# angelini/raft-simulation

Hardware: AMD Instinct MI355X
Metric: simulated node-ticks/sec (5-node Raft) (higher is better)
Workload: dtype u32; 1 GPU; C2: 65,536 5-node clusters/GPU, 10k ticks/step, no faults, no client (steady window); clusters=65536, clusters_per_gpu=65536, nodes=5, parallelism=cluster-sharded x1

## Files before the change

### raft-simulation_amd/csrc/steady_kernel.hip

```cpp
#include <hip/hip_ext.h>

#include "fixed_point_affine.hpp"
#include "tick_wave.hpp"

namespace rs {

constexpr int LANE_WG = 256;

__device__ __forceinline__ uint32_t msel(bool a, uint32_t x, uint32_t y) {
  const uint32_t m = 0u - (uint32_t)a;
  return (x & m) | (y & ~m);
}

constexpr int IMG_SLOTS = 32;
constexpr uint32_t IMG_LINE = 64 * 8 * 16;
constexpr uint32_t IMG_HALF = 2 * IMG_LINE;
constexpr uint32_t IMG_WAVE = 2 * IMG_HALF;
__device__ __forceinline__ uint32_t img_sw(uint32_t l) { return (l ^ (l >> 3)) & 7u; }
__device__ __forceinline__ uint32_t img_off(uint32_t l, uint32_t i) {
  return i < 16 ? (i >> 3) * IMG_LINE + l * 128u + 16u * ((i & 7u) ^ img_sw(l))
                : IMG_HALF + l * 256u + 16u * ((i & 15u) ^ (l & 15u));
}
template <typename T>
__device__ __forceinline__ T* lds_at(char* img, uint32_t off) {
// ... 49 lines not shown
  return SetWords{vreg(c.lead.a), vreg(c.lead.x), vreg(c.lead.y), vreg(c.lead.z),
                  vreg(c.fol.a),  vreg(c.fol.x),  vreg(c.fol.y),  vreg(c.fol.z),
                  vreg(c.lead.s), vreg(c.fol.s),  vreg(c.K),      vreg(K1)};
}
template <int I>
__device__ __forceinline__ void park_lane(uint32_t& park, uint32_t v) {
  asm volatile("v_writelane_b32 %0, %1, %2"
               : "+v"(park)
               : "s"(__builtin_amdgcn_readfirstlane(v)), "n"(I));
}
template <int F>
__device__ __forceinline__ fpa::Band band_sets(uint32_t nt, uint32_t d, uint32_t hb, BandSets* out) {
  const fpa::Band b = fpa::band(F, d, hb, nt);
  const uint32_t K1 = b.K1;
  const fpa::Set lo = fpa::build<F>(d, hb, K1 ? K1 - 1 : 0), hi = fpa::step<F>(lo, d, hb);
  out->k[0] = vreg(lo, K1);
  out->k[1] = vreg(hi, K1);
  return b;
}

template <int N>
struct FixedPoint {
  static constexpr int F = N - 1;
  static constexpr bool IN_BAND = false;
  uint32_t L, Lid, Lterm, Lcommit;
  uint64_t Ltr, ftr[F];
  uint32_t Ldl, fdl[F], fpend;
  uint32_t qmask, qA[F], qT[F], qa[F], qb[F];
  uint32_t rmask, resA, rT[F], rA[F], rB[F], rH[F];
  uint32_t nhb, nae, nar;

  __device__ __forceinline__ uint32_t fk(int j) const { return (uint32_t)j + ((uint32_t)j >= L ? 1u : 0u); }

  __device__ __forceinline__ void append_entries(uint32_t ta, uint32_t d, uint32_t el_base) {
#pragma unroll
    for (int j = 0; j < F; ++j) {
      ftr[j] = trace_event(ftr[j], ta, RAFT_MSG_APPEND_ENTRIES, Lid, Lterm, RAFT_FOLLWER, Lterm, 0);
      fdl[j] = ta + el_base;
      rT[j] = Lterm; rA[j] = Lcommit; rB[j] = 0; rH[j] = 1;
      qA[j] = INF;
    }
    fpend = (1u << F) - 1;
    qmask = 0;
    rmask = (1u << F) - 1;
    resA = ta + d;
    nae += F;
  }
  __device__ __forceinline__ void responses(uint32_t th, uint32_t tend, uint32_t d, uint32_t hb) {
#pragma unroll
    for (int j = 0; j < F; ++j) {
      const uint32_t tau = th + 2 * d + j;
      if (((rmask >> j) & 1) && tau < tend) {
        Ltr = trace_event(Ltr, tau, RAFT_MSG_APPEND_RESPONSE, fk(j) + 1, Lterm, RAFT_LEADER,
                          Lterm, 0);
        rmask &= ~(1u << j);
        Ldl = tau + hb;
        ++nar;
      }
    }
    if (!rmask) resA = INF;
  }
  __device__ __forceinline__ uint32_t term() const { return Lterm; }
  __device__ __forceinline__ uint32_t sid(int j) const { return fk(j) + 1; }
  __device__ __forceinline__ void followers(uint64_t a, uint64_t add) {
#pragma unroll
    for (int j = 0; j < F; ++j) ftr[j] = ftr[j] * a + add;
  }
  __device__ __forceinline__ void rearmed(uint32_t v) {
#pragma unroll
    for (int j = 0; j < F; ++j) fdl[j] = v;
    fpend = (1u << F) - 1;
  }
  __device__ __forceinline__ void heartbeat(uint32_t ta) {
#pragma unroll
    for (int j = 0; j < F; ++j) {
      qA[j] = ta; qT[j] = Lterm; qa[j] = Lcommit; qb[j] = 0;
    }
    qmask = (1u << F) - 1;
  }
  __device__ __forceinline__ bool queued() const { return rmask != 0; }

  __device__ __forceinline__ int slot(int k) const {
    return (uint32_t)k > L ? (k > 0 ? k - 1 : 0) : (k < F ? k : F - 1);
  }
  __device__ __forceinline__ uint32_t at_node(const uint32_t (&x)[F], int k) const {
    return msel((uint32_t)k > L, x[k > 0 ? k - 1 : 0], x[k < F ? k : F - 1]);
  }
  template <int NV>
  __device__ __forceinline__ void node_words(int k, uint32_t (&v)[NV][N]) const {
    const bool isL = (uint32_t)k == L;
    const int jl = k > 0 ? k - 1 : 0, jh = k < F ? k : F - 1;
    const bool lo = (uint32_t)k > L;
    const uint32_t fq = (qmask >> slot(k)) & 1, fqa = at_node(qA, k);
    const uint64_t trf = (uint64_t)msel(lo, (uint32_t)(ftr[jl] >> 32), (uint32_t)(ftr[jh] >> 32)) << 32 |
                         msel(lo, (uint32_t)ftr[jl], (uint32_t)ftr[jh]);
    const uint64_t tr = isL ? Ltr : trf;
    v[HF_DEADLINE][k] = isL ? Ldl : at_node(fdl, k);
    v[HF_TRACE_LO][k] = (uint32_t)tr;
    v[HF_TRACE_HI][k] = (uint32_t)(tr >> 32);
    v[HF_QMETA][k] = isL ? pack_qmeta(0, 0, 0, __popc(rmask)) : pack_qmeta(0, fq, 0, 0);
    v[HF_REQ_ARR][k] = isL ? INF : (fq ? fqa : INF);
    v[HF_RES_ARR][k] = isL ? resA : INF;
    v[HF_REQ_TAIL][k] = isL ? 0u : (fq ? fqa : 0u);
    v[HF_RES_TAIL][k] = isL ? (rmask ? resA : 0u) : 0u;
  }
  __device__ __forceinline__ void to_rings(const DevSim& S, uint32_t c, bool on) const {
    if (!__builtin_amdgcn_ballot_w64(on && (qmask || rmask))) return;
#pragma unroll
    for (int j = 0; j < F; ++j) {
      if (on && ((qmask >> j) & 1)) {
        uint4* dp = reinterpret_cast<uint4*>(qslots(S, c * N + fk(j), 0));
        dp[0] = make_uint4(qA[j], RAFT_MSG_APPEND_ENTRIES | Lid << 3, qT[j], qa[j]);
        dp[1] = make_uint4(qb[j], 0, 0, 0);
      }
    }
    uint4* rp = reinterpret_cast<uint4*>(qslots(S, c * N + L, 1));
    uint32_t n = 0;
#pragma unroll
    for (int j = 0; j < F; ++j) {
      if (on && ((rmask >> j) & 1)) {
        uint4* dp = rp + 2 * n;
        dp[0] = make_uint4(resA, RAFT_MSG_APPEND_RESPONSE | sid(j) << 3 | rH[j] << 7, rT[j], rA[j]);
        dp[1] = make_uint4(rB[j], 0, 0, 0);
        ++n;
      }
    }
  }
};

template <int N>
struct NodeOrder {
  static constexpr int F = N - 1;
  static constexpr bool IN_BAND = true;
  uint32_t L, T;
  uint64_t tr[N], Ltr;
  uint32_t Ldl;
  bool qin, took;
  uint32_t qA, fdl;
  uint32_t rc, resA;
  uint32_t nhb, nae, nar;

  __device__ __forceinline__ uint32_t sid(int j) const {
    return (uint32_t)j + 1 + ((uint32_t)j >= L ? 1u : 0u);
  }
  __device__ __forceinline__ void followers(uint64_t a, uint64_t add) {
#pragma unroll
    for (int k = 0; k < N; ++k) tr[k] = tr[k] * a + add;
  }
  __device__ __forceinline__ void append_entries(uint32_t ta, uint32_t d, uint32_t el_base) {
    followers(TRACE_M2, trace_term(ta, RAFT_MSG_APPEND_ENTRIES, L + 1, T, RAFT_FOLLWER, T, 0));
    took = true;
    fdl = ta + el_base;
    qin = false;
    rc = F;
    resA = ta + d;
    nae += F;
  }
  __device__ __forceinline__ void responses(uint32_t th, uint32_t tend, uint32_t d, uint32_t hb) {
#pragma unroll
    for (int j = 0; j < F; ++j) {
      const uint32_t tau = th + 2 * d + j;
      if ((uint32_t)j + rc >= (uint32_t)F && tau < tend) {
        Ltr = trace_event(Ltr, tau, RAFT_MSG_APPEND_RESPONSE, sid(j), T, RAFT_LEADER, T, 0);
        --rc;
        Ldl = tau + hb;
        ++nar;
      }
    }
    if (!rc) resA = INF;
  }
  __device__ __forceinline__ uint32_t term() const { return T; }
  __device__ __forceinline__ void rearmed(uint32_t v) { took = true; fdl = v; }
  __device__ __forceinline__ void heartbeat(uint32_t ta) { qin = true; qA = ta; }
  __device__ __forceinline__ bool queued() const { return rc != 0; }
};

struct LaunchBand {
  uint32_t t0;
  fpa::Band b;
};
template <typename St>
__device__ __forceinline__ void rounds(St& s, uint32_t th, uint32_t tend, uint32_t d, uint32_t hb,
                                       uint32_t el_base, const BandSets& bs, const LaunchBand& lb) {
  constexpr int F = St::F;
  const uint32_t P = 2 * d + F - 1 + hb, last = 2 * d + F - 1, T = s.term();
  uint32_t K, tk;
  if constexpr (St::IN_BAND) {
    const uint32_t delta = th - lb.t0;
    K = fpa::band_rounds(lb.b, delta);
    tk = th + fpa::band_ticks(lb.b, P, delta);
    const SetWords sw = bs.k[(delta <= lb.b.rho) & (lb.b.K1 != 0)];
    const fpa::Half cl = sw.lead(), cf = sw.fol();
    s.Ltr = fpa::apply_leader<F>(cl, s.Ltr, th, T, s.L);
    s.followers(cf.a, fpa::follower_addend<F>(cf, th, T, s.L));
    if (K) {
      s.rearmed(tk - P + d + el_base);
      s.Ldl = tk;
      s.nhb += K;
      s.nae += F * K;
      s.nar += F * K;
    }
  } else {
    K = tend > th + last ? (tend - th - last - 1) / P + 1 : 0;
    tk = th + K * P;
  }
  if (!St::IN_BAND && K) {
    const uint32_t K1 = bs.k[0].K1;
    const bool top = K == K1;
    if (!__builtin_amdgcn_ballot_w64(!top && K + 1 != K1)) {
      const SetWords sw = bs.k[top];
      const fpa::Half cl = sw.lead(), cf = sw.fol();
      s.Ltr = fpa::apply_leader<F>(cl, s.Ltr, th, T, s.L);
      s.followers(cf.a, fpa::follower_addend<F>(cf, th, T, s.L));
    } else {
      uint64_t a = trace_term(th, 7, 0, 0, RAFT_LEADER, T, 0);
#pragma unroll
      for (int j = 0; j < F; ++j)
        a = a * TRACE_M2 + trace_term(th + 2 * d + j, RAFT_MSG_APPEND_RESPONSE, s.sid(j), T,
                                      RAFT_LEADER, T, 0);
      const uint64_t da = (uint64_t)P * (TRACE_M * trace_geo<F + 1>());
      const uint64_t df = (uint64_t)P * TRACE_M;
      uint64_t cf = trace_term(th + d, RAFT_MSG_APPEND_ENTRIES, s.L + 1, T, RAFT_FOLLWER, T, 0);
      for (uint32_t r = 0; r < K; ++r) {
        s.Ltr = s.Ltr * trace_pow<F + 1>() + a;
        a += da;
        s.followers(TRACE_M2, cf);
        cf += df;
      }
    }
    s.rearmed(tk - P + d + el_base);
    s.Ldl = tk;
    s.nhb += K;
    s.nae += F * K;
    s.nar += F * K;
  }
  if (tk < tend) {
    s.Ltr = trace_event(s.Ltr, tk, 7, 0, 0, RAFT_LEADER, T, 0);
    ++s.nhb;
    s.Ldl = tk + hb;
    s.heartbeat(tk + d);
    if (tk + d < tend) {
      s.append_entries(tk + d, d, el_base);
      s.responses(tk, tend, d, hb);
    }
  }
}

template <typename St>
__device__ __forceinline__ void run_launch(St& s, uint32_t mid, uint32_t th0, uint32_t tend,
                                           uint32_t d, uint32_t hb, uint32_t el_base, uint32_t P,
                                           const BandSets& bs, const LaunchBand& lb) {
  bool whole = true;
  if (mid == 1) {
    if (th0 + d < tend) s.append_entries(th0 + d, d, el_base);
    else whole = false;
  }
  if (mid && whole) {
    s.responses(th0, tend, d, hb);
    whole = !s.queued();
  }
  if (whole) rounds(s, mid ? th0 + P : th0, tend, d, hb, el_base, bs, lb);
}

struct Schedule {
  uint32_t mid, th0, nxt;
  bool on;
};
template <int F>
__device__ __forceinline__ Schedule schedule(uint32_t t0, uint32_t tend, uint32_t d, uint32_t hb,
                                             uint32_t P, uint32_t Ldl, bool req, uint32_t reqA,
                                             uint32_t nres, uint32_t resA) {
  Schedule s{0, Ldl, 0, true};
  if (req) {
    s.mid = 1;
    s.th0 = reqA - d;
    s.on = reqA >= t0 && reqA >= d && Ldl == s.th0 + hb;
  } else if (nres) {
    s.mid = 2;
    s.th0 = resA - 2 * d;
    const uint32_t j0 = (uint32_t)F - nres;
    const int64_t cut = (int64_t)t0 - ((int64_t)s.th0 + 2 * d);
    s.on = resA >= 2 * d && (int64_t)j0 == (cut < 0 ? 0 : cut > F ? (int64_t)F : cut) &&
           Ldl == (j0 ? s.th0 + 2 * d + j0 - 1 : s.th0) + hb;
  } else {
    s.on = Ldl >= t0;
  }
  s.nxt = min((s.mid == 2 ? s.th0 + P : s.th0) + d, tend);
  return s;
}


template <int N>
__global__ void __launch_bounds__(LANE_WG) steady_lane_kernel(DevSim S, uint32_t t0, uint32_t nt) {
  static_assert(N >= 2 && N <= 5, "follower masks and the response queue fit four followers");
  constexpr int F = N - 1;
  constexpr uint32_t HB = hot_block_words(N);
  constexpr int NWORDS = (int)(HOT_CW + hf_abase(N) * N);
  constexpr int NW4 = (NWORDS + 3) / 4;
  constexpr int IMGC = (int)(HB / 4) < IMG_SLOTS ? (int)(HB / 4) : IMG_SLOTS;
  static_assert(NW4 <= IMGC && IMGC % 8 == 0, "the image holds the words read, in whole lines");
  __shared__ uint32_t bl_c[LANE_WG], bl_t[LANE_WG];
  __shared__ BandSets bs_keep[LANE_WG / 64];
  extern __shared__ __attribute__((aligned(16))) uint32_t dsm[];
  const uint32_t lane = threadIdx.x & 63, wave = threadIdx.x >> 6;
  const uint32_t cbase = blockIdx.x * LANE_WG + wave * 64;
  const uint32_t c0 = cbase + lane < S.C ? cbase + lane : INF;
  const bool active = c0 != INF;
  const uint32_t c = active ? c0 : 0u;
  const uint32_t g = S.goff + c;
  char* const img = reinterpret_cast<char*>(dsm) + wave * IMG_WAVE;
  uint32_t* const blc = bl_c + wave * 64;
  uint32_t* const blt = bl_t + wave * 64;
  uint32_t nbw = 0;
  auto record_bail = [&](bool b, uint32_t tick) {
    const uint64_t m = __builtin_amdgcn_ballot_w64(b);
    if (b) {
      const uint32_t i = nbw + __builtin_amdgcn_mbcnt_hi((uint32_t)(m >> 32),
                                                         __builtin_amdgcn_mbcnt_lo((uint32_t)m, 0u));
      blc[i] = c;
      blt[i] = tick;
    }
    nbw += (uint32_t)__popcll(m);
  };
#ifdef RS_WAVELOG
  const uint64_t wl_start = wall_clock64();
  uint32_t wl_trips = 0, wl_first = 0, wl_ph[6] = {0, 0, 0, 0, 0, 0};
  uint64_t wl_loop = 0, wl_ts = 0;
#define RS_LPH(i)                                         \
  do {                                                    \
    const uint64_t now_ = __builtin_amdgcn_s_memtime();   \
    wl_ph[i] += (uint32_t)(now_ - wl_ts);                 \
    wl_ts = now_;                                         \
  } while (0)
#else
#define RS_LPH(i) do {} while (0)
#endif

  auto load_wait = [&]() {
    asm volatile("s_waitcnt vmcnt(0)" ::: "memory");
  };
  auto load_line = [&](int ln, bool wait) {
    const uint32_t p = lane & 7;
#pragma unroll
    for (int j = 0; j < 8; ++j) {
      const uint32_t cc = 8 * j + (lane >> 3);
      const uint32_t i = 8 * ln + (p ^ img_sw(cc));
      const uint32_t cg = min(cbase + cc, S.C - 1);
      __builtin_amdgcn_global_load_lds(
          (const __attribute__((address_space(1))) void*)(S.hot + (size_t)cg * HB + 4 * i),
          (__attribute__((address_space(3))) void*)(img + ln * IMG_LINE + j * 1024), 16, 0, 0);
    }
    if (wait) load_wait();
  };
  auto load_half1 = [&]() {
    const uint32_t p = lane & 15;
#pragma unroll
    for (int j = 0; j < 16; ++j) {
      const uint32_t cc = 4 * j + (lane >> 4);
      const uint32_t i = 16 + (p ^ (cc & 15u));
      const uint32_t cg = min(cbase + cc, S.C - 1);
      if (i < (uint32_t)IMGC)
        __builtin_amdgcn_global_load_lds(
            (const __attribute__((address_space(1))) void*)(S.hot + (size_t)cg * HB + 4 * i),
            (__attribute__((address_space(3))) void*)(img + IMG_HALF + j * 1024), 16, 0, 0);
    }
    asm volatile("s_waitcnt vmcnt(0)" ::: "memory");
  };
  static_assert(IMGC >= 16, "lines 0 and 1 are whole in every block");
  uint32_t w[NW4 * 4];
  auto read_chunks = [&](int lo, int hi) {
#pragma unroll
    for (int i = lo; i < hi; ++i) {
      const uint4 x = *lds_at<const uint4>(img, img_off(lane, i));
      w[4 * i] = x.x; w[4 * i + 1] = x.y; w[4 * i + 2] = x.z; w[4 * i + 3] = x.w;
    }
  };
  auto word = [&](int f, int k) { return w[HOT_CW + f * N + k]; };
  auto lword = [&](int f, uint32_t L) {
    uint32_t v = 0;
#pragma unroll
    for (int k = 0; k < N; ++k) v |= word(f, k) & (0u - (uint32_t)(L == (uint32_t)k));
    return v;
  };
  auto fword = [&](int f, int j, uint32_t L) {
    return msel((uint32_t)j >= L, word(f, j + 1), word(f, j));
  };
  static_assert(HF_RES_TAIL + 1 == HF_FLAGS && (HOT_CW + HF_FLAGS * N) % 4 == 0 && HOT_CW % 4 == 0,
                "the fields written: DEADLINE .. RES_TAIL, whole chunks");
  constexpr int CH_END = (int)(HOT_CW + HF_FLAGS * N) / 4;
  asm volatile("" ::"s"(nt), "s"(t0), "s"(S.dmin), "s"(S.hb), "s"(S.el_base));
  load_line(0, false);
  const bool reporter = blockIdx.x == 0 && threadIdx.x == 0;
  uint32_t prev_bails = 0;
  if (reporter) prev_bails = *S.nbail_zero;
  uint32_t nt_s = nt;
  asm volatile("" : "+s"(nt_s));
  const BandSets& bs = bs_keep[wave];
  uint32_t park = 0;
  {
    const fpa::Band b = band_sets<F>(nt_s, S.dmin, S.hb, &bs_keep[wave]);
    park_lane<0>(park, b.K1);
    park_lane<1>(park, b.rho);
    park_lane<2>(park, b.K1P);
  }
  load_wait();
  asm volatile("" : "+v"(park));
  auto parked_band = [&]() {
    return fpa::Band{(uint32_t)__builtin_amdgcn_readlane(park, 0),
                     (uint32_t)__builtin_amdgcn_readlane(park, 1),
                     (uint32_t)__builtin_amdgcn_readlane(park, 2)};
  };
  if (reporter && prev_bails) {
    if (S.bail_report) *S.bail_report = prev_bails;
    *S.nbail_zero = 0;
  }
  static_assert(NW4 >= 8, "line 0 is read whole");
  read_chunks(0, 8);
  const uint32_t tend = t0 + nt, d = S.dmin, hb = S.hb, el_base = S.el_base;
  const uint32_t P = 2 * d + F - 1 + hb, allF = (1u << F) - 1;
  uint32_t dl = 0, nhb = 0, nae = 0, nar = 0;
  bool el = false;
  uint32_t el_to = 0;
#ifdef RS_WAVELOG
  uint64_t wl_x1 = 0, wl_x2 = 0, wl_x3 = 0, wl_lend = 0;
  uint32_t wl_cut = 0;
  asm volatile("" ::"v"(w[CL_CERT]), "v"(w[HOT_CW]));
  wl_loop = wall_clock64();
#endif

  static_assert(HOT_CW + (HF_QMETA + 1) * N <= 32 && HF_DEADLINE < HF_QMETA &&
                    HF_TRACE_LO < HF_QMETA && HF_TRACE_HI < HF_QMETA && CL_CTERM < HOT_CW,
                "every word the line-0 path reads is in line 0; REQ_ARR, RES_ARR, the flags and "
                "the term are derived (device.hpp)");
  NodeOrder<N> no;
  uint32_t lmid = 0, lth0 = 0;
  const bool cfg_ok = el_base >= P && hb >= 2 * d + F && S.Q >= (uint32_t)F;
  bool strong = active & cfg_ok & ((w[CL_CERT] & 0xFFFF0000u) == CERT_STRONG) &
                ((w[CL_CERT] & 0xFFFFu) < (uint32_t)N);
  {
    const uint32_t L = w[CL_CERT] & 0xFFFFu;
    no.L = L; no.T = w[CL_CTERM];
    no.Ldl = lword(HF_DEADLINE, L);
    no.Ltr = (uint64_t)lword(HF_TRACE_HI, L) << 32 | lword(HF_TRACE_LO, L);
#pragma unroll
    for (int k = 0; k < N; ++k) no.tr[k] = (uint64_t)word(HF_TRACE_HI, k) << 32 | word(HF_TRACE_LO, k);
    no.took = false; no.fdl = 0;
    no.nhb = no.nae = no.nar = 0;
    const uint32_t Lqm = lword(HF_QMETA, L), rsc = qm_res_cnt(Lqm);
    const uint32_t qm0 = L ? word(HF_QMETA, 0) : word(HF_QMETA, 1);
    const bool need = qm0 != 0;
    const bool cutr = !need & (rsc != 0);
    const uint32_t one_req = pack_qmeta(0, 1, 0, 0), only_res = pack_qmeta(0, 0, 0, rsc);
    strong = strong & ((qm0 & ~one_req) == 0) & (Lqm == only_res) & (rsc <= (uint32_t)F) &
             !(need & (rsc != 0));
#pragma unroll
    for (int k = 0; k < N; ++k) strong = strong & ((L == (uint32_t)k) | (word(HF_QMETA, k) == qm0));
    const uint32_t j0 = (uint32_t)F - rsc;
    const uint32_t back = msel(need | cutr, hb + msel(cutr & (j0 != 0), 2 * d + j0 - 1, 0u), 0u);
    lmid = msel(need, 1u, msel(cutr, 2u, 0u));
    lth0 = no.Ldl - back;
    const uint32_t ta = lth0 + d, ra = lth0 + 2 * d;
    const int64_t cut = (int64_t)t0 - (int64_t)ra;
    const bool on_need = ta >= t0;
    const bool on_cut = (int64_t)j0 == (cut < 0 ? 0 : cut > F ? (int64_t)F : cut);
    const bool on_none = no.Ldl >= t0;
    strong = strong & (no.Ldl >= back) & (need ? on_need : cutr ? on_cut : on_none);
    no.qin = need;
    no.qA = msel(need, ta, 0u);
    no.rc = msel(cutr, rsc, 0u);
    no.resA = msel(cutr, ra, INF);
    const uint32_t nxt = min(msel(cutr, lth0 + P, lth0) + d, tend);
#pragma unroll
    for (int k = 0; k < N; ++k)
      strong = strong & ((L == (uint32_t)k) | (word(HF_DEADLINE, k) >= nxt));
    strong = strong & (msel(lmid != 0, lth0 + P, lth0) - t0 < P);
  }
  const bool line0_wave = !__builtin_amdgcn_ballot_w64(active && !strong);
  if (line0_wave) {
#ifdef RS_WAVELOG
    asm volatile("" ::"v"(no.Ltr), "v"(no.Ldl), "v"(no.tr[0]), "v"(lth0));
    wl_x1 = wl_x2 = wall_clock64();
#endif
    if (active) {
      const LaunchBand lb{t0, parked_band()};
      run_launch(no, lmid, lth0, tend, d, hb, el_base, P, bs, lb);
      nhb = no.nhb; nae = no.nae; nar = no.nar;
#ifdef RS_WAVELOG
      asm volatile("" ::"v"(no.Ltr), "v"(no.tr[0]), "v"(no.Ldl));
      wl_x3 = wall_clock64();
#endif
      const uint32_t fqm = pack_qmeta(0, no.qin ? 1u : 0u, 0, 0), Lqm = pack_qmeta(0, 0, 0, no.rc);
      const uint32_t fra = no.qin ? no.qA : INF, frt = no.qin ? no.qA : 0u;
      const uint32_t Lrt = no.rc ? no.resA : 0u;
      auto val = [&](int q) -> uint32_t {
        const int f = (q - (int)HOT_CW) / N, k = (q - (int)HOT_CW) % N;
        const bool isL = no.L == (uint32_t)k;
        switch (f) {
          case HF_DEADLINE: return isL ? no.Ldl : no.took ? no.fdl : w[q];
          case HF_TRACE_LO: return (uint32_t)(isL ? no.Ltr : no.tr[k]);
          case HF_TRACE_HI: return (uint32_t)((isL ? no.Ltr : no.tr[k]) >> 32);
          case HF_QMETA: return isL ? Lqm : fqm;
          case HF_REQ_ARR: return isL ? INF : fra;
          case HF_RES_ARR: return isL ? no.resA : INF;
          case HF_REQ_TAIL: return isL ? 0u : frt;
          default: return isL ? Lrt : 0u;
        }
      };
      auto chunk = [&](int i) {
        return make_uint4(val(4 * i), val(4 * i + 1), val(4 * i + 2), val(4 * i + 3));
      };
#pragma unroll
      for (int i = (int)HOT_CW / 4; i < (CH_END < 8 ? CH_END : 8); ++i)
        *lds_at<uint4>(img, img_off(lane, i)) = chunk(i);
      dl = (nhb | nae | nar) != 0;
      if (CH_END > 8 && (lmid || no.qin || no.rc)) {
        uint4* const bp = reinterpret_cast<uint4*>(S.hot + (size_t)c * HB);
#pragma unroll
        for (int i = 8; i < CH_END; ++i) bp[i] = chunk(i);
      }
    }
    if (__builtin_amdgcn_ballot_w64(active && (no.qin || no.rc))) {
      if (active && no.qin) {
#pragma unroll
        for (int k = 0; k < N; ++k) {
          if (no.L != (uint32_t)k) {
            uint4* dp = reinterpret_cast<uint4*>(qslots(S, c * N + k, 0));
            dp[0] = make_uint4(no.qA, RAFT_MSG_APPEND_ENTRIES | (no.L + 1) << 3, no.T, 0);
            dp[1] = make_uint4(0, 0, 0, 0);
          }
        }
      }
      uint4* rp = reinterpret_cast<uint4*>(qslots(S, c * N + no.L, 1));
      uint32_t n = 0;
#pragma unroll
      for (int j = 0; j < F; ++j) {
        if (active && (uint32_t)j + no.rc >= (uint32_t)F) {
          uint4* dp = rp + 2 * n;
          dp[0] = make_uint4(no.resA, RAFT_MSG_APPEND_RESPONSE | no.sid(j) << 3 | 1u << 7, no.T, 0);
          dp[1] = make_uint4(0, 0, 0, 0);
          ++n;
        }
      }
    }
#ifdef RS_WAVELOG
    wl_lend = wall_clock64();
    wl_cut = __builtin_amdgcn_ballot_w64(active && (lmid || no.qin || no.rc)) ? 1u : 0u;
#endif
  }

  uint32_t Lc = 0;
  bool cert = false, full = false;
  if (!line0_wave) {
    load_line(1, true);
#pragma unroll
    for (int i = 32; i < NW4 * 4; ++i) w[i] = 0;
    read_chunks(8, NW4 < 16 ? NW4 : 16);
    uint32_t nlc = 0;
#pragma unroll
    for (int k = 0; k < N; ++k) {
      const bool lead = fl_role(w[HOT_CW + HF_FLAGS * N + k]) == RAFT_LEADER;
      Lc = lead ? (uint32_t)k : Lc;
      nlc += lead;
    }
    static_assert(HOT_CW + (HF_FLAGS + 1) * N <= 64, "the flags are in the first two lines");
    cert = active && nlc == 1 &&
           (w[CL_CERT] == (CERT_MAGIC | Lc) || w[CL_CERT] == (CERT_STRONG | Lc));
    full = IMGC > 16 && __builtin_amdgcn_ballot_w64(active && !cert) != 0;
    if (full) {
      load_half1();
      read_chunks(16, NW4);
    }
  }
  const bool vouched = cert && !full;

  FixedPoint<N> fx;
  const LaunchBand no_band{t0, fpa::Band{0, 0, 0}};
  bool lean = false;
  if (!line0_wave) {
    lean = vouched && cfg_ok;
    const uint32_t L = Lc;
    fx.L = L; fx.Lid = L + 1; fx.Lterm = lword(HF_TERM, L); fx.Lcommit = 0;
    fx.Ldl = lword(HF_DEADLINE, L);
    fx.Ltr = (uint64_t)lword(HF_TRACE_HI, L) << 32 | lword(HF_TRACE_LO, L);
    fx.qmask = fx.rmask = 0; fx.resA = INF; fx.fpend = allF; fx.nhb = fx.nae = fx.nar = 0;
    const uint32_t Lqm = lword(HF_QMETA, L);
    const uint32_t rsc = qm_res_cnt(Lqm);
    uint32_t need = 0;
#pragma unroll
    for (int j = 0; j < F; ++j) {
      fx.fdl[j] = fword(HF_DEADLINE, j, L);
      fx.ftr[j] = (uint64_t)fword(HF_TRACE_HI, j, L) << 32 | fword(HF_TRACE_LO, j, L);
      const uint32_t qm = fword(HF_QMETA, j, L);
      lean = lean && (fword(HF_FLAGS, j, L) & FL_DRAW) && ((qm >> 4) & 31) <= 1 && !qm_res_cnt(qm);
      need |= (qm_req_cnt(qm) ? 1u : 0u) << j;
      fx.qA[j] = INF; fx.qT[j] = fx.qa[j] = fx.qb[j] = 0;
      fx.rT[j] = fx.rA[j] = fx.rB[j] = fx.rH[j] = 0;
    }
    lean = lean && !qm_req_cnt(Lqm) && rsc <= (uint32_t)F && !(need && rsc) &&
           (need == 0 || need == allF);
    const uint32_t ta = fword(HF_REQ_ARR, 0, L), ra = lword(HF_RES_ARR, L);
    const Schedule sc = schedule<F>(t0, tend, d, hb, P, fx.Ldl, need != 0, ta, rsc, ra);
    lean = lean && sc.on;
    lmid = sc.mid;
    lth0 = sc.th0;
    if (lmid == 1) {
#pragma unroll
      for (int j = 0; j < F; ++j) {
        lean = lean && fword(HF_REQ_ARR, j, L) == ta;
        fx.qA[j] = ta; fx.qT[j] = fx.Lterm;
      }
      fx.qmask = allF;
    } else if (lmid == 2) {
      fx.rmask = allF & ~((1u << ((uint32_t)F - rsc)) - 1);
      fx.resA = ra;
#pragma unroll
      for (int j = 0; j < F; ++j) {
        fx.rT[j] = fx.Lterm; fx.rH[j] = 1;
      }
    }
#pragma unroll
    for (int j = 0; j < F; ++j) lean = lean && fx.fdl[j] >= sc.nxt;
  }
  const bool lean_wave = !line0_wave && !__builtin_amdgcn_ballot_w64(active && !lean);
  bool wb = false;
  if (lean_wave) {
#ifdef RS_WAVELOG
    asm volatile("" ::"v"(fx.Ltr), "v"(fx.fdl[0]), "v"(fx.ftr[0]), "v"(lth0));
    wl_x1 = wl_x2 = wall_clock64();
#endif
    if (active) {
      run_launch(fx, lmid, lth0, tend, d, hb, el_base, P, bs, no_band);
      nhb = fx.nhb; nae = fx.nae; nar = fx.nar;
#ifdef RS_WAVELOG
      asm volatile("" ::"v"(fx.Ltr), "v"(fx.ftr[0]), "v"(fx.Ldl));
      wl_x3 = wall_clock64();
#endif
      uint32_t v[HF_FLAGS][N];
#pragma unroll
      for (int k = 0; k < N; ++k) fx.node_words(k, v);
      auto val = [&](int q) { return v[(q - HOT_CW) / N][(q - HOT_CW) % N]; };
      auto chunk = [&](int i) {
        return make_uint4(val(4 * i), val(4 * i + 1), val(4 * i + 2), val(4 * i + 3));
      };
#pragma unroll
      for (int i = (int)HOT_CW / 4; i < CH_END; ++i) {
        const int q = 4 * i;
        const uint4 x = chunk(i);
        *lds_at<uint4>(img, img_off(lane, i)) = x;
        dl |= (uint32_t)(x.x != w[q] || x.y != w[q + 1] || x.z != w[q + 2] || x.w != w[q + 3])
              << (i / 8);
      }
      const uint32_t cn = CERT_STRONG | fx.L;
      *lds_at<uint4>(img, img_off(lane, CL_CERT / 4)) =
          make_uint4(w[CL_CERT - 3], w[CL_CERT - 2], fx.Lterm, cn);
      static_assert(CL_CTERM == CL_CERT - 1 && CL_CERT % 4 == 3, "one chunk");
      dl |= (uint32_t)(cn != w[CL_CERT] || fx.Lterm != w[CL_CTERM]);
    }
    fx.to_rings(S, c, active);
#ifdef RS_WAVELOG
    wl_lend = wall_clock64();
#endif
  } else if (!line0_wave) {
#ifdef RS_WAVELOG
    wl_loop = wall_clock64();
#endif
    {
      auto ifield = [&](int f, int k) { return w[HOT_CW + f * N + k]; };
      bool pat = active && w[CL_HWM_IDX] == 0 && S.Q >= 2u * F && el_base >= P && hb >= 2 * d + F;
      const uint32_t T = ifield(HF_TERM, 0);
#pragma unroll
      for (int k = 0; k < N; ++k) {
        pat = pat && ifield(HF_FLAGS, k) == 0 && ifield(HF_MASKS, k) == 0 &&
              ifield(HF_TERM, k) == T && ifield(HF_COMMIT, k) == 0 && ifield(HF_LEN, k) == 0 &&
              ifield(HF_QMETA, k) == 0 && ifield(HF_REQ_ARR, k) == INF &&
              ifield(HF_RES_ARR, k) == INF;
#pragma unroll
        for (int p = 0; p < 2 * N; ++p) pat = pat && ifield(HF_NEXT + p, k) == 0;
      }
      pat = pat && T != INF;
      uint32_t cidx = 0, t1 = INF, ntie = 0, bidx = 0;
#pragma unroll
      for (int k = 0; k < N; ++k) {
        const uint32_t dk = ifield(HF_DEADLINE, k);
        cidx = dk < t1 ? (uint32_t)k : cidx;
        t1 = min(t1, dk);
      }
      bool single = true;
#pragma unroll
      for (int k = 0; k < N; ++k) {
        const uint32_t dk = ifield(HF_DEADLINE, k);
        ntie += dk == t1;
        bidx = dk == t1 && (uint32_t)k != cidx ? (uint32_t)k : bidx;
        single = single && ((uint32_t)k == cidx || (uint64_t)dk >= (uint64_t)t1 + d);
      }
      const bool tie = ntie == 2 && d == 1 && N >= 3;
      constexpr uint32_t iL = (N + 1) / 2 >= 2 ? (N + 1) / 2 - 2 : 0;
      const uint64_t tL = (uint64_t)t1 + 2 * d + iL;
      const uint64_t tau0 = max((uint64_t)t1 + 2 * d + F, tL + 2 * d);
      const uint64_t tlast = tau0 + F - 1;
      pat = pat && (single || tie) && t1 >= t0 && (tie || tlast < tend) &&
            (uint64_t)t1 + 4 * N + 8 < 0xFFFFFFFFull;
      if (__builtin_amdgcn_ballot_w64(pat)) {
        const uint32_t* lp = S.hot + (size_t)c * HB + HOT_CW + hf_led(N) * N;
        uint32_t led[N];
#pragma unroll
        for (int k = 0; k < N; ++k) led[k] = lp[k];
#pragma unroll
        for (int k = 0; k < N; ++k) pat = pat && ((uint32_t)k == cidx || led[k] != T + 1);
      }
      const uint32_t T1 = T + 1, cid = cidx + 1, peers = ((1u << (N + 1)) - 1) & ~1u & ~(1u << cid);
      if (pat && single) {
        el = true;
        el_to = 1;
        uint64_t hc = 0;
#pragma unroll
        for (int k = 0; k < N; ++k)
          if ((uint32_t)k == cidx)
            hc = (uint64_t)ifield(HF_TRACE_HI, k) << 32 | ifield(HF_TRACE_LO, k);
        hc = trace_event(hc, t1, 6, 0, 0, RAFT_CANDIDATE, T1, 0);
#pragma unroll
        for (int i = 0; i < F; ++i) {
          const uint32_t sid = (uint32_t)i + ((uint32_t)i >= cidx ? 2u : 1u);
          hc = trace_event(hc, t1 + 2 * d + i, RAFT_MSG_VOTE_RESPONSE, sid, T,
                           (uint32_t)i >= iL ? RAFT_LEADER : RAFT_CANDIDATE, T1, 0);
        }
#pragma unroll
        for (int j = 0; j < F; ++j) {
          const uint32_t sid = (uint32_t)j + ((uint32_t)j >= cidx ? 2u : 1u);
          hc = trace_event(hc, (uint32_t)tau0 + j, RAFT_MSG_APPEND_RESPONSE, sid, T, RAFT_LEADER,
                           T1, 0);
        }
#pragma unroll
        for (int k = 0; k < N; ++k) {
          const bool isc = (uint32_t)k == cidx;
          uint64_t h = (uint64_t)ifield(HF_TRACE_HI, k) << 32 | ifield(HF_TRACE_LO, k);
          h = trace_event(h, t1 + d, RAFT_MSG_REQUEST_VOTE, cid, T1, RAFT_FOLLOWER, T, 0);
          h = trace_event(h, (uint32_t)tL + d, RAFT_MSG_APPEND_ENTRIES, cid, T1, RAFT_FOLLWER, T1, 0);
          h = isc ? hc : h;
          w[HOT_CW + HF_FLAGS * N + k] = isc ? pack_flags(RAFT_LEADER, 0, cid, 0, 0, 1)
                                             : pack_flags(RAFT_FOLLWER, 0, cid, 0, 0, 0) | FL_DRAW;
          w[HOT_CW + HF_MASKS * N + k] = isc ? peers << 16 : 0u;
          w[HOT_CW + HF_TERM * N + k] = T1;
          w[HOT_CW + HF_DEADLINE * N + k] = isc ? (uint32_t)tlast + hb
                                                : (uint32_t)tL + d + el_base;
          w[HOT_CW + HF_REQ_TAIL * N + k] = 0;
          w[HOT_CW + HF_RES_TAIL * N + k] = 0;
          w[HOT_CW + HF_TRACE_LO * N + k] = (uint32_t)h;
          w[HOT_CW + HF_TRACE_HI * N + k] = (uint32_t)(h >> 32);
        }
        nae = F;
        nar = F;
      } else if (pat && tie) {
        const uint32_t a = cidx, b = bidx, B = b + 1;
        const uint32_t A = cid;
        constexpr uint32_t M = (N + 1) / 2;
        uint64_t ha = 0, hbb = 0;
#pragma unroll
        for (int k = 0; k < N; ++k) {
          const uint64_t h0 = (uint64_t)ifield(HF_TRACE_HI, k) << 32 | ifield(HF_TRACE_LO, k);
          if ((uint32_t)k == a) ha = h0;
          if ((uint32_t)k == b) hbb = h0;
        }
        ha = trace_event(ha, t1, 6, 0, 0, RAFT_CANDIDATE, T1, 0);
        ha = trace_event(ha, t1 + 1, RAFT_MSG_REQUEST_VOTE, B, T1, RAFT_CANDIDATE, T1, 0);
        uint32_t votes = 1, tLt = INF, role = RAFT_CANDIDATE;
#pragma unroll
        for (int k = 0; k < N; ++k) {
          if ((uint32_t)k == a) continue;
          const uint32_t i = (uint32_t)k - ((uint32_t)k > a ? 1u : 0u), tau = t1 + 2 + i;
          const bool grant = (uint32_t)k != b;
          if (grant && role == RAFT_CANDIDATE && ++votes >= M) {
            role = RAFT_LEADER;
            tLt = tau;
          }
          ha = trace_event(ha, tau, RAFT_MSG_VOTE_RESPONSE, (uint32_t)k + 1, grant ? T : T1, role,
                           T1, 0);
        }
        hbb = trace_event(hbb, t1, 6, 0, 0, RAFT_CANDIDATE, T1, 0);
        hbb = trace_event(hbb, t1 + 1, RAFT_MSG_REQUEST_VOTE, A, T1, RAFT_CANDIDATE, T1, 0);
        hbb = trace_event(hbb, t1 + 2, RAFT_MSG_VOTE_RESPONSE, A, T1, RAFT_CANDIDATE, T1, 0);
        uint32_t tb = t1 + 3, j = 0, tbae = INF, brole = RAFT_CANDIDATE, bdl = 0;
        bool bexact = false;
        for (int it = 0; it < N + 1; ++it) {
          const bool res = j < (uint32_t)N - 2, req = tbae == INF;
          if (!res && !req) break;
          if (!res && tb < tLt + 1) tb = tLt + 1;
          const bool rq = req && tb >= tLt + 1;
          bool take_req = rq;
          bexact = false;
          if (res && rq) {
            const uint4 ew = event_draw(g, B, tb, S);
            take_req = !(ew.x & 1);
            bexact = true;
            bdl = tb + el_base + __umulhi(ew.y, S.el_span);
          }
          if (take_req) {
            hbb = trace_event(hbb, tb, RAFT_MSG_APPEND_ENTRIES, A, T1, RAFT_FOLLWER, T1, 0);
            brole = RAFT_FOLLWER;
            tbae = tb;
          } else {
            uint32_t fid = 0, cnt = 0;
#pragma unroll
            for (int k = 0; k < N; ++k) {
              const bool other = (uint32_t)k != a && (uint32_t)k != b;
              fid = other && cnt == j ? (uint32_t)k + 1 : fid;
              cnt += other;
            }
            hbb = trace_event(hbb, tb, RAFT_MSG_VOTE_RESPONSE, fid, T, brole, T1, 0);
            ++j;
          }
          if (!bexact) bdl = tb + el_base;
          ++tb;
        }
        const uint32_t tbl = tb - 1;
        uint32_t ta = t1 + N + 1;
        const uint32_t fa = tLt + 2, ba = tbae + 1;
#pragma unroll
        for (int k = 0; k < N; ++k) {
          if ((uint32_t)k == a) continue;
          const bool isb = (uint32_t)k == b;
          if (isb && ba != fa) continue;
          ta = max(ta, fa);
          ha = trace_event(ha, ta, RAFT_MSG_APPEND_RESPONSE, (uint32_t)k + 1, isb ? T1 : T,
                           RAFT_LEADER, T1, 0);
          ++ta;
        }
        if (ba != fa) {
          ta = max(ta, ba);
          ha = trace_event(ha, ta, RAFT_MSG_APPEND_RESPONSE, B, T1, RAFT_LEADER, T1, 0);
          ++ta;
        }
        const uint32_t tal = ta - 1;
        if (tbae != INF && tLt != INF && max(tal, tbl) < tend) {
          el = true;
          el_to = 2;
#pragma unroll
          for (int k = 0; k < N; ++k) {
            const bool isa = (uint32_t)k == a, isb = (uint32_t)k == b;
            uint64_t h = (uint64_t)ifield(HF_TRACE_HI, k) << 32 | ifield(HF_TRACE_LO, k);
            h = trace_event(h, t1 + 1, RAFT_MSG_REQUEST_VOTE, A, T1, RAFT_FOLLOWER, T, 0);
            h = trace_event(h, t1 + 2, RAFT_MSG_REQUEST_VOTE, B, T1, RAFT_FOLLOWER, T, 0);
            h = trace_event(h, tLt + 1, RAFT_MSG_APPEND_ENTRIES, A, T1, RAFT_FOLLWER, T1, 0);
            h = isa ? ha : isb ? hbb : h;
            w[HOT_CW + HF_FLAGS * N + k] =
                isa ? pack_flags(RAFT_LEADER, 0, A, 0, 0, 1)
                    : pack_flags(RAFT_FOLLWER, 0, A, 0, 0, 0) | (isb && bexact ? 0u : FL_DRAW);
            w[HOT_CW + HF_MASKS * N + k] = isa ? peers << 16 : 0u;
            w[HOT_CW + HF_TERM * N + k] = T1;
            w[HOT_CW + HF_DEADLINE * N + k] = isa ? tal + hb : isb ? bdl : tLt + 1 + el_base;
            w[HOT_CW + HF_REQ_TAIL * N + k] = 0;
            w[HOT_CW + HF_RES_TAIL * N + k] = 0;
            w[HOT_CW + HF_TRACE_LO * N + k] = (uint32_t)h;
            w[HOT_CW + HF_TRACE_HI * N + k] = (uint32_t)(h >> 32);
          }
          nae = F;
          nar = F;
        }
      }
    }
    uint32_t L = 0, nlead = 0, badn = 0;
#pragma unroll
    for (int k = 0; k < N; ++k) {
      const uint32_t f = word(HF_FLAGS, k);
      const bool lead = fl_role(f) == RAFT_LEADER;
      L = lead ? (uint32_t)k : L;
      nlead += lead;
      badn |= fl_fault(f) | (lead != (fl_lsp(f) != 0)) | (lead && (f & FL_DRAW));
    }
    bool bad = !active || nlead != 1 || badn != 0 || S.Q < (uint32_t)F;
    const uint32_t Lid = L + 1;
    const uint32_t Lfl = lword(HF_FLAGS, L), Lterm = lword(HF_TERM, L);
    const uint32_t Lcommit = lword(HF_COMMIT, L), Llen = lword(HF_LEN, L);
    uint32_t Lmk = lword(HF_MASKS, L);
    fx.L = L; fx.Lid = Lid; fx.Lterm = Lterm; fx.Lcommit = Lcommit;
    fx.Ldl = lword(HF_DEADLINE, L);
    fx.Ltr = (uint64_t)lword(HF_TRACE_HI, L) << 32 | lword(HF_TRACE_LO, L);
    fx.nhb = nhb; fx.nae = nae; fx.nar = nar;
    uint32_t ffl[F], fmk[F], fterm[F], fcommit[F], flen[F];
    int32_t nx[F], mt[F], nx0[F], mt0[F];
#pragma unroll
    for (int j = 0; j < F; ++j) {
      ffl[j] = fword(HF_FLAGS, j, L);
      fmk[j] = fword(HF_MASKS, j, L);
      fterm[j] = fword(HF_TERM, j, L);
      fcommit[j] = fword(HF_COMMIT, j, L);
      flen[j] = fword(HF_LEN, j, L);
      fx.fdl[j] = fword(HF_DEADLINE, j, L);
      fx.ftr[j] = (uint64_t)fword(HF_TRACE_HI, j, L) << 32 | fword(HF_TRACE_LO, j, L);
      const bool up = (uint32_t)j >= L;
      nx[j] = nx0[j] = (int32_t)msel(up, lword(HF_NEXT + j + 1, L), lword(HF_NEXT + j, L));
      mt[j] = mt0[j] = (int32_t)msel(up, lword(HF_NEXT + N + j + 1, L), lword(HF_NEXT + N + j, L));
    }
    const bool ackbad = Llen > w[CL_HWM_IDX];
    const uint32_t Lkeys = Lmk >> 16;
    bad = bad || (Lkeys & (((1u << (N + 1)) - 1) & ~1u & ~(1u << Lid))) !=
                     (((1u << (N + 1)) - 1) & ~1u & ~(1u << Lid)) ||
          (Lfl & FL_SEQ) || Lcommit > Llen;

#ifdef RS_WAVELOG
    asm volatile("" ::"v"(fx.Ltr), "v"(fx.fdl[0]), "v"(nx[0]));
    wl_x1 = wall_clock64();
#endif
    fx.qmask = 0; fx.rmask = 0; fx.resA = INF;
#pragma unroll
    for (int j = 0; j < F; ++j) {
      fx.qA[j] = INF; fx.qT[j] = fx.qa[j] = fx.qb[j] = 0;
      fx.rT[j] = fx.rA[j] = fx.rB[j] = fx.rH[j] = 0;
    }
    if (!bad) {
      const uint32_t Lqm = lword(HF_QMETA, L);
      bad = qm_req_cnt(Lqm);
      const uint32_t rsh = qm_res_head(Lqm), rsc = qm_res_cnt(Lqm);
      uint32_t need = 0, rqh[F];
#pragma unroll
      for (int j = 0; j < F; ++j) {
        const uint32_t qm = fword(HF_QMETA, j, L);
        const uint32_t rqc = qm_req_cnt(qm);
        rqh[j] = qm_req_head(qm);
        bad = bad || rqc > 1 || qm_res_cnt(qm) != 0;
        need |= (uint32_t)(rqc != 0) << j;
      }
      bad = bad || rsc > (uint32_t)F;
      uint4 qm0[F], qm1[F], rm0[F], rm1[F];
      if (__builtin_amdgcn_ballot_w64(!bad && (need || rsc))) {
#pragma unroll
        for (int j = 0; j < F; ++j) {
          const uint4* mp = reinterpret_cast<const uint4*>(
              qslots(S, c * N + fx.fk(j), 0) + min(rqh[j], S.Q - 1) * qstride(S, 0));
          qm0[j] = mp[0];
          qm1[j] = mp[1];
        }
#pragma unroll
        for (int i = 0; i < F; ++i) {
          const uint4* mp = reinterpret_cast<const uint4*>(
              qslots(S, c * N + L, 1) + min(wrapq(rsh + i, S.Q), S.Q - 1) * qstride(S, 1));
          rm0[i] = mp[0];
          rm1[i] = mp[1];
        }
      }
      if (!bad) {
#pragma unroll
        for (int j = 0; j < F; ++j) {
          if ((need >> j) & 1) {
            const uint4 m0 = qm0[j], m1 = qm1[j];
            bad = bad || m0.y != (RAFT_MSG_APPEND_ENTRIES | Lid << 3) || m1.y || m1.z || m1.w;
            fx.qmask |= 1u << j;
            fx.qA[j] = m0.x; fx.qT[j] = m0.z; fx.qa[j] = m0.w; fx.qb[j] = m1.x;
          }
        }
        uint32_t last = 0;
#pragma unroll
        for (int i = 0; i < F; ++i) {
          if ((uint32_t)i < rsc && !bad) {
            const uint4 m0 = rm0[i], m1 = rm1[i];
            const uint32_t hdr = m0.y, src = (hdr >> 3) & 15;
            bad = (hdr & 7) != RAFT_MSG_APPEND_RESPONSE || (hdr >> 8) || m1.y || m1.z || m1.w ||
                  src <= last || src > (uint32_t)N || src == Lid || (i && m0.x != fx.resA);
            last = src;
            fx.resA = m0.x;
// ... 472 lines not shown
```

Before: 570600 billion node-ticks/s.

## Use scalar base addressing for full-wave line loads and trim cut-path stores

Makes the wave index wave-uniform and adds a fast path for full waves in load_line, where the per-slot global address is a scalar base plus a lane XOR offset, which reduces per-lane address arithmetic. The cut path now writes constant idle values for the hot block when no queue or response is pending, and writes request and response queue slots through direct pointer arithmetic without zeroing the upper half of each slot. That zeroing moves to the fixed-point certificate path, which clears it once per cluster. The change depends on the hot-block and queue layout assumptions (HB a multiple of 32, the qbuf stride) staying valid.

New measurement: 569000 billion node-ticks/s. About the same (-0.3%).

```diff
diff --git a/raft-simulation_amd/csrc/steady_kernel.hip b/raft-simulation_amd/csrc/steady_kernel.hip
--- a/raft-simulation_amd/csrc/steady_kernel.hip
+++ b/raft-simulation_amd/csrc/steady_kernel.hip
@@ -375,7 +375,7 @@
   __shared__ uint32_t bl_c[LANE_WG], bl_t[LANE_WG];
   __shared__ BandSets bs_keep[LANE_WG / 64];
   extern __shared__ __attribute__((aligned(16))) uint32_t dsm[];
-  const uint32_t lane = threadIdx.x & 63, wave = threadIdx.x >> 6;
+  const uint32_t lane = threadIdx.x & 63, wave = __builtin_amdgcn_readfirstlane(threadIdx.x >> 6);
   const uint32_t cbase = blockIdx.x * LANE_WG + wave * 64;
   const uint32_t c0 = cbase + lane < S.C ? cbase + lane : INF;
   const bool active = c0 != INF;
@@ -412,8 +412,24 @@
   auto load_wait = [&]() {
     asm volatile("s_waitcnt vmcnt(0)" ::: "memory");
   };
+  static_assert(HB % 32 == 0, "blocks are whole lines: a slot's XOR stays inside its line");
   auto load_line = [&](int ln, bool wait) {
     const uint32_t p = lane & 7;
+    if (cbase + 64 <= S.C) {
+      const uint32_t r = lane >> 3, off0 = r * (HB * 4) + 16u * (p ^ r);
+      const char* const sb = reinterpret_cast<const char*>(S.hot + (size_t)cbase * HB) + ln * 128;
+#pragma unroll
+      for (int j = 0; j < 8; ++j) {
+        uint64_t sbj = reinterpret_cast<uint64_t>(sb) + (uint64_t)j * (8 * HB * 4);
+        asm volatile("" : "+s"(sbj));
+        __builtin_amdgcn_global_load_lds(
+            (const __attribute__((address_space(1))) void*)(reinterpret_cast<const char*>(sbj) +
+                                                            (off0 ^ (16u * j))),
+            (__attribute__((address_space(3))) void*)(img + ln * IMG_LINE + j * 1024), 16, 0, 0);
+      }
+      if (wait) load_wait();
+      return;
+    }
 #pragma unroll
     for (int j = 0; j < 8; ++j) {
       const uint32_t cc = 8 * j + (lane >> 3);
@@ -588,30 +604,49 @@
       dl = (nhb | nae | nar) != 0;
       if (CH_END > 8 && (lmid || no.qin || no.rc)) {
         uint4* const bp = reinterpret_cast<uint4*>(S.hot + (size_t)c * HB);
-#pragma unroll
-        for (int i = 8; i < CH_END; ++i) bp[i] = chunk(i);
+        if (!no.qin && !no.rc) {
+          auto idle = [](int q) -> uint32_t {
+            const int f = (q - (int)HOT_CW) / N;
+            return f == HF_REQ_ARR || f == HF_RES_ARR ? INF : 0u;
+          };
+#pragma unroll
+          for (int i = 8; i < CH_END; ++i)
+            bp[i] = make_uint4(idle(4 * i), idle(4 * i + 1), idle(4 * i + 2), idle(4 * i + 3));
+        } else {
+          const uint32_t lm = 0u - (uint32_t)(no.rc != 0);
+          auto cutv = [&](int q) -> uint32_t {
+            const int f = (q - (int)HOT_CW) / N, k = (q - (int)HOT_CW) % N;
+            const bool isL = no.L == (uint32_t)k;
+            switch (f) {
+              case HF_REQ_ARR: return isL ? INF : fra;
+              case HF_RES_ARR: return isL ? no.resA : INF;
+              case HF_REQ_TAIL: return isL ? 0u : frt;
+              default: return isL ? no.resA & lm : 0u;
+            }
+          };
+#pragma unroll
+          for (int i = 8; i < CH_END; ++i)
+            bp[i] = make_uint4(cutv(4 * i), cutv(4 * i + 1), cutv(4 * i + 2), cutv(4 * i + 3));
+        }
       }
     }
     if (__builtin_amdgcn_ballot_w64(active && (no.qin || no.rc))) {
       if (active && no.qin) {
-#pragma unroll
-        for (int k = 0; k < N; ++k) {
-          if (no.L != (uint32_t)k) {
-            uint4* dp = reinterpret_cast<uint4*>(qslots(S, c * N + k, 0));
-            dp[0] = make_uint4(no.qA, RAFT_MSG_APPEND_ENTRIES | (no.L + 1) << 3, no.T, 0);
-            dp[1] = make_uint4(0, 0, 0, 0);
-          }
-        }
-      }
-      uint4* rp = reinterpret_cast<uint4*>(qslots(S, c * N + no.L, 1));
-      uint32_t n = 0;
-#pragma unroll
-      for (int j = 0; j < F; ++j) {
-        if (active && (uint32_t)j + no.rc >= (uint32_t)F) {
-          uint4* dp = rp + 2 * n;
-          dp[0] = make_uint4(no.resA, RAFT_MSG_APPEND_RESPONSE | no.sid(j) << 3 | 1u << 7, no.T, 0);
-          dp[1] = make_uint4(0, 0, 0, 0);
-          ++n;
+        char* const rq = reinterpret_cast<char*>(S.qbuf) + (size_t)c * (N * 32);
+        const uint4 m = make_uint4(no.qA, RAFT_MSG_APPEND_ENTRIES | (no.L + 1) << 3, no.T, 0);
+#pragma unroll
+        for (int j = 0; j < F; ++j)
+          *reinterpret_cast<uint4*>(rq + 32 * j + ((uint32_t)j >= no.L ? 32u : 0u)) = m;
+      }
+      if (active && no.rc) {
+        const uintptr_t rp =
+            reinterpret_cast<uintptr_t>(S.qbuf) +
+            ((size_t)S.Q * S.NN + ((size_t)c * N + no.L) * S.Q + no.rc) * 32 - (size_t)F * 32;
+#pragma unroll
+        for (int j = 0; j < F; ++j) {
+          if ((uint32_t)j + no.rc >= (uint32_t)F)
+            *reinterpret_cast<uint4*>(rp + 32 * j) =
+                make_uint4(no.resA, RAFT_MSG_APPEND_RESPONSE | no.sid(j) << 3 | 1u << 7, no.T, 0);
         }
       }
     }
@@ -728,6 +763,16 @@
           make_uint4(w[CL_CERT - 3], w[CL_CERT - 2], fx.Lterm, cn);
       static_assert(CL_CTERM == CL_CERT - 1 && CL_CERT % 4 == 3, "one chunk");
       dl |= (uint32_t)(cn != w[CL_CERT] || fx.Lterm != w[CL_CTERM]);
+      {
+        const uint4 z = make_uint4(0, 0, 0, 0);
+        char* const rq = reinterpret_cast<char*>(S.qbuf) + (size_t)c * (N * 32) + 16;
+        char* const rs = reinterpret_cast<char*>(qslots(S, c * N + fx.L, 1)) + 16;
+#pragma unroll
+        for (int j = 0; j < F; ++j) {
+          *reinterpret_cast<uint4*>(rq + 32 * fx.fk(j)) = z;
+          *reinterpret_cast<uint4*>(rs + 32 * j) = z;
+        }
+      }
     }
     fx.to_rings(S, c, active);
 #ifdef RS_WAVELOG
```
